# Atif-Anwer/SHMGAN

Hardware: AMD Instinct MI355X
Metric: images/sec (gen+disc train_step) (higher is better)
Workload: dtype f32; 1 GPU; SHMGAN train_step 256x256 5-view, batch 8/GPU, filter_size 64, fp32 (BASELINE configs[1]); global_batch=8, image_size=256, parallelism=dp1, losses_finite=True

## Files before the change

### shmgan_amd/csrc/conv_halo.hip

```cpp
#include "tapgemm_dev.h"

template <typename T, typename TO, int BN, int PH = 16, bool ST = false, int TM = 2, bool GS = false, int NM = 0>
__global__ __launch_bounds__(BN * PH / (2 * TM), ST ? BN * PH / (256 * TM) : 1) void tapgemm_halo_kernel(const TapGemmArgs a) {
    static_assert(TM == 2 || (TM == 4 && ST), "four M tiles per wave: static-tap form only");
    static_assert(!NM || (ST && TM == 2 && !GS), "norm: static-tap forward form");
    constexpr int ESZ = sizeof(T), CHE = 16 / ESZ, BKE = 64 / ESZ;
    constexpr int WGM = PH / (2 * TM), WGN = BN / 64, NW = WGM * WGN;
    constexpr int HC = 18, NIT = PH == 16 ? 24 : 12;
    constexpr int NHR = NIT * 16;
    constexpr int ASTG = NHR * 16, BSTG = BN * 16;
    constexpr int NA = NIT / NW, NB = (BN / 16) / NW;
    static_assert(NIT % NW == 0 && (BN / 16) % NW == 0, "DMA items divide over the waves");
    __shared__ __attribute__((aligned(1024))) float smem[2 * ASTG + 3 * BSTG];
    __shared__ __attribute__((aligned(1024))) float snt[NM ? SHM_NT_PLANES * SHM_NT_MAXC : 4];
    float* const sA = smem;
    float* const sB = smem + 2 * ASTG;
    typedef __attribute__((address_space(3))) void* lds_ptr;

    const TapPhase& P = a.ph[0];
    const int tid = threadIdx.x;
    const int lane = tid & 63, wave = __builtin_amdgcn_readfirstlane(tid >> 6);
    const int l31 = lane & 31, h = lane >> 5;
    const int wm = wave / WGN, wn = wave % WGN;
    const int ppr = a.wi >> 4, ppi = (a.hi / PH) * ppr;
    const int img = blockIdx.x / ppi, prem = blockIdx.x - img * ppi;
    const int y0 = (prem / ppr) * PH, x0 = (prem % ppr) << 4;
    const int n0 = blockIdx.y * BN;
    [[maybe_unused]] const bool nm_table = NM == 1 || (NM == 2 && (y0 == 0 || y0 + PH == a.hi || x0 == 0 || x0 + 16 == a.wi));

    const int drow = lane >> 2, dq = lane & 3;
    unsigned arow1[NA], arow2[NA];
    [[maybe_unused]] int nmv[NA];
#pragma unroll
    for (int j = 0; j < NA; ++j) {
        const int hrow = 16 * (wave + NW * j) + drow;
        const int hr = hrow / HC, hc = hrow - hr * HC;
        const int iy = y0 - 1 + hr, ix = x0 - 1 + hc;
        const bool v = hrow < (PH + 2) * HC && (unsigned)iy < (unsigned)a.hi && (unsigned)ix < (unsigned)a.wi;
        const int pix = (img * a.hi + iy) * a.wi + ix;
        const int coff = (dq ^ (ST ? ((hrow >> 1) + hr) & 3 : (hrow >> 2) & 3)) * CHE;
        arow1[j] = v ? (unsigned)(pix * a.ldx + coff) * (unsigned)ESZ : 0xffffffffu;
        arow2[j] = v ? (unsigned)(pix * a.ldx2 + coff) * (unsigned)ESZ : 0xffffffffu;
        nmv[j] = v ? coff : hrow < (PH + 2) * HC ? -1 - coff : (int)0x80000000;
    }
    unsigned wrow[NB];
#pragma unroll
    for (int j = 0; j < NB; ++j) {
        const int row = (wave + NW * j) * 16 + drow;
        const int nn = n0 + row;
        wrow[j] = nn < a.nout ? (unsigned)(nn * a.K + (dq ^ ((row >> 2) & 3)) * CHE) * (unsigned)ESZ : 0xffffffffu;
    }
    const __amdgpu_buffer_rsrc_t rsx = __builtin_amdgcn_make_buffer_rsrc((void*)a.x, 0, a.xbytes, 0x00020000);
    const __amdgpu_buffer_rsrc_t rsx2 = __builtin_amdgcn_make_buffer_rsrc((void*)a.x2, 0, a.x2bytes, 0x00020000);
    const __amdgpu_buffer_rsrc_t rsw = __builtin_amdgcn_make_buffer_rsrc((void*)a.w, 0, a.wbytes, 0x00020000);

    const int nch = a.K / BKE;
    const int ksteps = 9 * nch;
    const int tl = lane < 9 ? lane : 0;
    const int tapsh_v = P.dh[tl] * HC + P.dw[tl];
    const int tapw_v = P.widx[tl];

    auto dma_a = [&](int chunk) {
        const int c0 = chunk * BKE;
        const bool second = c0 >= a.c1;
        const unsigned cb = (unsigned)(second ? c0 - a.c1 : c0) * (unsigned)ESZ;
        float* dst = sA + (chunk & 1) * ASTG + wave * 256;
#pragma unroll
        for (int j = 0; j < NA; ++j) {
            const unsigned r = second ? arow2[j] : arow1[j];
            const unsigned off = r == 0xffffffffu ? r : r + cb;
            if (second)
                __builtin_amdgcn_raw_ptr_buffer_load_lds(rsx2, (lds_ptr)(dst + j * NW * 256), 16, (int)off, 0, 0, 0);
            else
                __builtin_amdgcn_raw_ptr_buffer_load_lds(rsx, (lds_ptr)(dst + j * NW * 256), 16, (int)off, 0, 0, 0);
        }
    };
    int ld_tap = 0, ld_chunk = 0, ld_stage = 0;
    auto dma_b = [&]() {
        const int t_wi = __builtin_amdgcn_readlane(tapw_v, ld_tap);
        const unsigned wbase = (unsigned)((t_wi * a.nout) * a.K + ld_chunk * BKE) * (unsigned)ESZ + (NM == 2 ? (unsigned)img * a.wimg : 0u);
#pragma unroll
        for (int j = 0; j < NB; ++j) {
            const unsigned off = wrow[j] == 0xffffffffu ? wrow[j] : wrow[j] + wbase;
            __builtin_amdgcn_raw_ptr_buffer_load_lds(rsw, (lds_ptr)(sB + ld_stage * BSTG + (wave + NW * j) * 256), 16, (int)off, 0, 0, 0);
        }
        if (++ld_tap == 9) {
            ld_tap = 0;
            ++ld_chunk;
        }
        ld_stage = ld_stage == 2 ? 0 : ld_stage + 1;
    };

    f32x16 acc[TM][2];
#pragma unroll
    for (int i = 0; i < TM; ++i)
#pragma unroll
        for (int j = 0; j < 2; ++j)
#pragma unroll
            for (int r = 0; r < 16; ++r) acc[i][j][r] = 0.f;

    int hb[TM];
#pragma unroll
    for (int i = 0; i < TM; ++i) hb[i] = (2 * TM * wm + 2 * i + (l31 >> 4) + 1) * HC + (l31 & 15) + 1;
    const int swb = (l31 >> 2) & 3;
    const int fb0 = l31 * 16 + ((0 + h) ^ swb) * 4, fb1 = l31 * 16 + ((2 + h) ^ swb) * 4;

    [[maybe_unused]] f32x4 abl_frag = {0.f, 0.f, 0.f, 0.f};
    if constexpr (abl::nolds) abl_frag = *(const f32x4*)(sA + lane * 4);
    auto compute = [&](int chunk, int tap, int bstage) {
        const float* Ab = sA + (chunk & 1) * ASTG;
        const float* Bb = sB + bstage * BSTG + wn * 64 * 16;
        const int sh = __builtin_amdgcn_readlane(tapsh_v, tap);
        int fa[2][2];
#pragma unroll
        for (int i = 0; i < 2; ++i) {
            const int hrow = hb[i] + sh;
            const int sw = (hrow >> 2) & 3;
            fa[i][0] = hrow * 16 + ((0 + h) ^ sw) * 4;
            fa[i][1] = hrow * 16 + ((2 + h) ^ sw) * 4;
        }
#pragma unroll
        for (int kk = 0; kk < 2; ++kk) {
            f32x4 av[2], bv[2];
            if constexpr (abl::nolds) {
                for (int i = 0; i < 2; ++i) av[i] = abl_frag;
                for (int j = 0; j < 2; ++j) bv[j] = abl_frag;
                asm volatile("" : "+v"(av[0]), "+v"(av[1]), "+v"(bv[0]), "+v"(bv[1]));
            } else {
#pragma unroll
                for (int i = 0; i < 2; ++i) av[i] = *(const f32x4*)(Ab + fa[i][kk]);
#pragma unroll
                for (int j = 0; j < 2; ++j) bv[j] = *(const f32x4*)(Bb + j * 512 + (kk ? fb1 : fb0));
            }
            if constexpr (TM == 2) tap_mfma<T, 2, 2>(av, bv, acc);
        }
    };

    [[maybe_unused]] int ntc_s = NM ? a.ntc : 0;
    if constexpr (NM != 0) asm volatile("" : "+s"(ntc_s));
    [[maybe_unused]] auto norm_a = [&](int chunk) {
        const int c0 = chunk * BKE;
        const bool second = c0 >= a.c1;
        if ((int)second != a.ntpart) return;
        const float* tb0 = snt + (second ? c0 - a.c1 : c0);
        float* dst = sA + (chunk & 1) * ASTG + wave * 256 + lane * 4;
        if constexpr (NM == 2) {
            if (!nm_table) return;
#pragma unroll
            for (int j = 0; j < NA; ++j) {
                const int m = nmv[j];
                if (m < 0 && m != (int)0x80000000) {
                    const float* tb = tb0 + (-1 - m) + 3 * ntc_s;
                    float* p = dst + j * NW * 256;
                    if constexpr (ESZ == 4) {
                        *(f32x4*)p = *(const f32x4*)tb;
                    } else {
                        const f32x4 r0 = *(const f32x4*)tb, r1 = *(const f32x4*)(tb + 4);
                        u32x4 x;
#pragma unroll
                        for (int e = 0; e < 2; ++e) {
                            x[e] = (unsigned)__builtin_bit_cast(unsigned short, (bf16_t)r0[2 * e]) |
                                   ((unsigned)__builtin_bit_cast(unsigned short, (bf16_t)r0[2 * e + 1]) << 16);
                            x[2 + e] = (unsigned)__builtin_bit_cast(unsigned short, (bf16_t)r1[2 * e]) |
                                       ((unsigned)__builtin_bit_cast(unsigned short, (bf16_t)r1[2 * e + 1]) << 16);
                        }
                        *(u32x4*)p = x;
                    }
                }
            }
            return;
        } else {
#pragma unroll
        for (int j = 0; j < NA; ++j) {
            if (nmv[j] >= 0) {
                const float* tb = tb0 + nmv[j];
                float* p = dst + j * NW * 256;
                if constexpr (ESZ == 4) {
                    f32x4 x = *(const f32x4*)p;
                    const f32x4 mean = *(const f32x4*)tb, inv = *(const f32x4*)(tb + ntc_s), beta = *(const f32x4*)(tb + 2 * ntc_s);
#pragma unroll
                    for (int e = 0; e < 4; ++e) x[e] = shm_in_norm(x[e], mean[e], inv[e], beta[e]);
                    *(f32x4*)p = x;
                } else {
                    u32x4 x = *(const u32x4*)p;
#pragma unroll
                    for (int hf = 0; hf < 2; ++hf) {
                        const f32x4 mean = *(const f32x4*)(tb + 4 * hf), inv = *(const f32x4*)(tb + ntc_s + 4 * hf),
                                    beta = *(const f32x4*)(tb + 2 * ntc_s + 4 * hf);
#pragma unroll
                        for (int e = 0; e < 2; ++e) {
                            const unsigned u = x[2 * hf + e];
                            const bf16_t lo = (bf16_t)shm_in_norm(__uint_as_float(u << 16), mean[2 * e], inv[2 * e], beta[2 * e]);
                            const bf16_t hi = (bf16_t)shm_in_norm(__uint_as_float(u & 0xffff0000u), mean[2 * e + 1], inv[2 * e + 1], beta[2 * e + 1]);
                            x[2 * hf + e] = (unsigned)__builtin_bit_cast(unsigned short, lo) | ((unsigned)__builtin_bit_cast(unsigned short, hi) << 16);
                        }
                    }
                    *(u32x4*)p = x;
                }
            }
        }
        }
    };

    if constexpr (NM) if (nm_table) {
        const __amdgpu_buffer_rsrc_t rsn = __builtin_amdgcn_make_buffer_rsrc((void*)a.nt, 0, a.ntbytes, 0x00020000);
        if (wave < SHM_NT_PLANES)
            __builtin_amdgcn_raw_ptr_buffer_load_lds(rsn, (lds_ptr)(snt + wave * 256), 16,
                                                     (int)((unsigned)img * 16u * (unsigned)a.ntc + (unsigned)wave * 1024u + (unsigned)lane * 16u), 0, 0, 0);
    }
    dma_a(0);
    dma_b();
    if (ksteps > 1) dma_b();
    if constexpr (NM) if (nm_table) {
        asm volatile("s_waitcnt vmcnt(%0)" ::"n"(2 * NB) : "memory");
        SHM_LDS_BARRIER();
        asm volatile("" ::: "memory");
        norm_a(0);
    }
    if constexpr (ST) {
        int fs[9];
#pragma unroll
        for (int t = 0; t < 9; ++t) {
            const int hrow = hb[0] + P.dh[t] * HC + P.dw[t];
            fs[t] = hrow * 16 + ((h ^ (((hrow >> 1) + hrow / HC) & 3)) << 2);
        }
        typedef const __attribute__((address_space(3))) f32x4* lds_f4;
        const unsigned sA_lds = (unsigned)(size_t)(__attribute__((address_space(3))) float*)sA;
        int tw[9];
#pragma unroll
        for (int t = 0; t < 9; ++t) tw[t] = __builtin_amdgcn_readlane(tapw_v, t);
        auto dma_b_at = [&](int t_wi, int chunk2, int stage2) {
            const unsigned wbase = (unsigned)((t_wi * a.nout) * a.K + chunk2 * BKE) * (unsigned)ESZ + (NM == 2 ? (unsigned)img * a.wimg : 0u);
#pragma unroll
            for (int j = 0; j < NB; ++j) {
                const unsigned off = wrow[j] == 0xffffffffu ? wrow[j] : wrow[j] + wbase;
                __builtin_amdgcn_raw_ptr_buffer_load_lds(rsw, (lds_ptr)(sB + stage2 * BSTG + (wave + NW * j) * 256), 16, (int)off, 0, 0, 0);
            }
        };
        for (int chunk = 0; chunk < nch; ++chunk) {
            const unsigned Ab = sA_lds + (unsigned)((chunk & 1) * ASTG * 4);
#pragma unroll
            for (int tap = 0; tap < 9; ++tap) {
                if (tap == 8 && chunk + 1 == nch)
                    asm volatile("s_waitcnt vmcnt(0)" ::: "memory");
                else if (tap == 1 && chunk + 1 < nch)
                    asm volatile("s_waitcnt vmcnt(%0)" ::"n"(NA + NB) : "memory");
                else
                    asm volatile("s_waitcnt vmcnt(%0)" ::"n"(NB) : "memory");
                SHM_LDS_BARRIER();
                asm volatile("" ::: "memory");
                if constexpr (!abl::nodma) {
                    if (tap == 0 && chunk + 1 < nch) dma_a(chunk + 1);
                    if (tap < 7 || chunk + 1 < nch) dma_b_at(tw[(tap + 2) % 9], chunk + (tap + 2) / 9, (tap + 2) % 3);
                }
                const float* Bb = sB + (tap % 3) * BSTG + wn * 64 * 16;
#pragma unroll
                for (int kk = 0; kk < 2; ++kk) {
                    f32x4 av[TM], bv[2];
                    if constexpr (abl::nolds) {
                        for (int i = 0; i < TM; ++i) av[i] = abl_frag;
                        for (int j = 0; j < 2; ++j) bv[j] = abl_frag;
                        asm volatile("" : "+v"(av[0]), "+v"(av[1]), "+v"(bv[0]), "+v"(bv[1]));
                    } else {
                        const lds_f4 ap = (lds_f4)(size_t)((Ab + (unsigned)(fs[tap] << 2)) ^ (unsigned)(kk << 5));
#pragma unroll
                        for (int i = 0; i < TM; ++i) av[i] = ap[i * (2 * HC * 4)];
#pragma unroll
                        for (int j = 0; j < 2; ++j) bv[j] = *(const f32x4*)(Bb + j * 512 + (kk ? fb1 : fb0));
                    }
                    if constexpr (!abl::nomfma)
                        tap_mfma<T, TM, 2>(av, bv, acc);
                    else
                        asm volatile("" :: "v"(av[0]), "v"(av[1]), "v"(bv[0]), "v"(bv[1]));
                }
                asm volatile("" ::: "memory");
                if constexpr (NM)
                    if (tap == 2 && chunk + 1 < nch && nm_table) {
                        norm_a(chunk + 1);
                        asm volatile("" ::: "memory");
                    }
            }
        }
    } else {
    int tap = 0, chunk = 0, bst = 0;
    for (int s = 0; s < ksteps; ++s) {
        if (s + 1 < ksteps) {
            if (tap == 1 && chunk + 1 < nch)
                asm volatile("s_waitcnt vmcnt(%0)" ::"n"(NA + NB) : "memory");
            else
                asm volatile("s_waitcnt vmcnt(%0)" ::"n"(NB) : "memory");
        } else {
            asm volatile("s_waitcnt vmcnt(0)" ::: "memory");
        }
        SHM_LDS_BARRIER();
        asm volatile("" ::: "memory");
        if constexpr (!abl::nodma) {
            if (tap == 0 && chunk + 1 < nch) dma_a(chunk + 1);
            if (s + 2 < ksteps) dma_b();
        }
        if constexpr (!abl::nomfma) compute(chunk, tap, bst);
        asm volatile("" ::: "memory");
        bst = bst == 2 ? 0 : bst + 1;
        if (++tap == 9) {
            tap = 0;
            ++chunk;
        }
    }
    }

    float s1[2], s2[2];
#pragma unroll
    for (int j = 0; j < 2; ++j) s1[j] = s2[j] = 0.f;
    float bj[2];
#pragma unroll
    for (int j = 0; j < 2; ++j) {
        const int n = n0 + wn * 64 + j * 32 + l31;
        bj[j] = (a.bias && n < a.nout) ? a.bias[(NM == 2 ? (size_t)img * a.bias_img : (size_t)0) + n] : 0.f;
        asm volatile("" : "+v"(bj[j]));
    }
    constexpr bool kWide = sizeof(TO) == 2;
    const bool wide = kWide && (a.nout % 8 == 0) && (a.n1 % 8 == 0) && (a.ldy % 8 == 0) && (((size_t)a.y & 15) == 0) &&
                      (a.y2 == nullptr || ((a.ldy2 % 8 == 0) && (((size_t)a.y2 & 15) == 0)));
    if constexpr (kWide) if (wide) {
        __syncthreads();
        unsigned short* tile = (unsigned short*)smem + wave * (TM * 32 * 64);
#pragma unroll
        for (int i = 0; i < TM; ++i) {
#pragma unroll
            for (int r = 0; r < 16; ++r) {
                const int row = i * 32 + (r & 3) + 8 * (r >> 2) + 4 * h;
#pragma unroll
                for (int j = 0; j < 2; ++j) {
                    const int n = n0 + wn * 64 + j * 32 + l31;
                    float v = acc[i][j][r] + bj[j];
                    const TO vo = (TO)shm_lrelu(v, a.slope);
                    v = n < a.nout ? (float)vo : 0.f;
                    s1[j] += v;
                    s2[j] = __builtin_fmaf(v, v, s2[j]);
                    const int col = j * 32 + l31;
                    tile[row * 64 + ((((col >> 3) ^ (row & 7)) << 3) | (col & 7))] = __builtin_bit_cast(unsigned short, vo);
                }
            }
        }
        asm volatile("s_waitcnt lgkmcnt(0)" ::: "memory");
        const int rr = lane >> 3, ch = lane & 7;
        const int n = n0 + wn * 64 + ch * 8;
        const int gp = __builtin_amdgcn_readfirstlane(n0 + wn * 64) < a.n1 ? 0 : 1;
        const int gpc = gp ? a.nout - a.n1 : a.n1, gnl = n - (gp ? a.n1 : 0);
        const bool gon = GS && a.gred[gp] != nullptr;
        const bool gs = gon && n < a.nout;
        const __amdgpu_buffer_rsrc_t rsa = __builtin_amdgcn_make_buffer_rsrc((void*)a.gaux[gp], 0, gon ? 0xfffffff0u : 0u, 0x00020000);
        const unsigned ldab = (unsigned)a.ldgaux[gp] * 2u;
        float t1[8], t2[8];
        u32x4 gav[4 * TM];
        if constexpr (GS) {
#pragma unroll
            for (int e = 0; e < 8; ++e) t1[e] = t2[e] = 0.f;
#pragma unroll
            for (int it = 0; it < 4 * TM; ++it) {
                const int row = it * 8 + rr;
                const int i = row >> 5, r32 = row & 31;
                const int py = 2 * TM * wm + 2 * i + (r32 >> 4), px = r32 & 15;
                const unsigned opix = (unsigned)((img * a.hi + (y0 + py)) * a.wi + (x0 + px));
                gav[it] = __builtin_bit_cast(u32x4, __builtin_amdgcn_raw_buffer_load_b128(rsa, opix * ldab + (unsigned)(n < a.nout ? gnl : 0) * 2u, 0, 0));
            }
            asm volatile("" ::: "memory");
        }
#pragma unroll
        for (int it = 0; it < 4 * TM; ++it) {
            const int row = it * 8 + rr;
            const u32x4 v = *(const u32x4*)(tile + row * 64 + ((ch ^ (row & 7)) << 3));
            const int i = row >> 5, r32 = row & 31;
            const int py = 2 * TM * wm + 2 * i + (r32 >> 4), px = r32 & 15;
            const size_t opix = ((size_t)img * a.hi + (y0 + py)) * a.wi + (x0 + px);
            if (!abl::nostore && n < a.nout) {
                if (n < a.n1)
                    *(u32x4*)((unsigned short*)a.y + opix * a.ldy + n) = v;
                else
                    *(u32x4*)((unsigned short*)a.y2 + opix * a.ldy2 + (n - a.n1)) = v;
            }
            if constexpr (GS) {
                gsum_wide_accum(v, gav[it], t1, t2);
                asm volatile("" ::: "memory");
            }
        }
        if constexpr (GS) {
            if (gon) {
                const int slot = (prem * WGM + wm) % a.gslots;
                double* dst = gs ? a.gred[gp] + ((size_t)slot * a.gbatch * gpc + (size_t)img * gpc + gnl) * 2 : nullptr;
                gsum_wide_flush<8>(t1, t2, lane, dst);
            }
        }
    }
    const bool gs_any = GS && sizeof(TO) == 4 && (a.gred[0] != nullptr || a.gred[1] != nullptr);
    if constexpr (GS && sizeof(TO) == 4) if (!wide && gs_any) {
#pragma unroll
        for (int j = 0; j < 2; ++j) {
            const int nb = __builtin_amdgcn_readfirstlane(n0 + wn * 64 + j * 32);
            const int gp = nb < a.n1 ? 0 : 1;
            const bool on = a.gred[gp] != nullptr && nb < a.nout;
            const int n = nb + l31;
            const int nl = n - (gp ? a.n1 : 0);
            const int pc = gp ? a.nout - a.n1 : a.n1;
            const __amdgpu_buffer_rsrc_t rsa = __builtin_amdgcn_make_buffer_rsrc((void*)a.gaux[gp], 0, on ? 0xfffffff0u : 0u, 0x00020000);
            const unsigned ldab = (unsigned)a.ldgaux[gp] * (unsigned)sizeof(T), nlb = (unsigned)(n < a.nout ? nl : 0) * (unsigned)sizeof(T);
            const __amdgpu_buffer_rsrc_t rsy = __builtin_amdgcn_make_buffer_rsrc(gp ? a.y2 : a.y, 0, gp ? a.y2bytes : a.ybytes, 0x00020000);
            const unsigned ldyb = (unsigned)(gp ? a.ldy2 : a.ldy) * (unsigned)sizeof(TO), nyb = (unsigned)(n < a.nout ? nl : 0) * (unsigned)sizeof(TO);
#pragma unroll
            for (int i = 0; i < TM; ++i) {
                const unsigned pix0 = (unsigned)((img * a.hi + (y0 + 2 * TM * wm + 2 * i)) * a.wi + x0 + 4 * h);
                const unsigned ao = pix0 * ldab + nlb, yo = pix0 * ldyb + nyb;
                float q[16];
#pragma unroll
                for (int r = 0; r < 16; ++r) {
                    const unsigned cr = (unsigned)((r >> 3) * a.wi + 8 * ((r >> 2) & 1) + (r & 3));
                    if constexpr (sizeof(T) == 4)
                        q[r] = __builtin_bit_cast(float, __builtin_amdgcn_raw_buffer_load_b32(rsa, ao, cr * ldab, 0));
                    else
                        q[r] = __uint_as_float((unsigned)__builtin_amdgcn_raw_buffer_load_b16(rsa, ao, cr * ldab, 0) << 16);
                }
                if (n < a.nout) {
#pragma unroll
                    for (int r = 0; r < 16; ++r) {
                        const unsigned cr = (unsigned)((r >> 3) * a.wi + 8 * ((r >> 2) & 1) + (r & 3));
                        float v = acc[i][j][r] + bj[j];
                        const TO vo = (TO)shm_lrelu(v, a.slope);
                        v = (float)vo;
                        s1[j] += v;
                        s2[j] += v * q[r];
                        __builtin_amdgcn_raw_buffer_store_b32(__builtin_bit_cast(unsigned, vo), rsy, yo, cr * ldyb, 0);
                    }
                }
            }
            if (on) {
                const int slot = (prem * WGM + wm) % a.gslots;
                const float t1 = s1[j] + __shfl_xor(s1[j], 32, 64);
                const float t2 = s2[j] + __shfl_xor(s2[j], 32, 64);
                if (h == 0 && n < a.nout) {
                    double* dst = a.gred[gp] + ((size_t)slot * a.gbatch * pc + (size_t)img * pc + nl) * 2;
                    atomicAdd(dst, (double)t1);
                    atomicAdd(dst + 1, (double)t2);
                }
            }
        }
    }
    const bool ybuf = !abl::nostore && a.ybytes != 0 && (a.y2 == nullptr || (a.y2bytes != 0 && a.n1 % 32 == 0));
    if (!wide && !gs_any && ybuf) {
#pragma unroll
        for (int j = 0; j < 2; ++j) {
            const int nb = __builtin_amdgcn_readfirstlane(n0 + wn * 64 + j * 32);
            const int gp = nb < a.n1 ? 0 : 1;
            const int n = nb + l31;
            const __amdgpu_buffer_rsrc_t rsy = __builtin_amdgcn_make_buffer_rsrc(gp ? a.y2 : a.y, 0, gp ? a.y2bytes : a.ybytes, 0x00020000);
            const unsigned ldyb = (unsigned)(gp ? a.ldy2 : a.ldy) * (unsigned)sizeof(TO);
            const unsigned nyb = (unsigned)(n < a.nout ? n - (gp ? a.n1 : 0) : 0) * (unsigned)sizeof(TO);
            if (n < a.nout) {
#pragma unroll
                for (int i = 0; i < TM; ++i) {
                    const unsigned yo = (unsigned)((img * a.hi + (y0 + 2 * TM * wm + 2 * i)) * a.wi + x0 + 4 * h) * ldyb + nyb;
#pragma unroll
                    for (int r = 0; r < 16; ++r) {
                        const unsigned cr = (unsigned)((r >> 3) * a.wi + 8 * ((r >> 2) & 1) + (r & 3));
                        float v = acc[i][j][r] + bj[j];
                        const TO vo = (TO)shm_lrelu(v, a.slope);
                        v = (float)vo;
                        s1[j] += v;
                        s2[j] = __builtin_fmaf(v, v, s2[j]);
                        if constexpr (sizeof(TO) == 4)
                            __builtin_amdgcn_raw_buffer_store_b32(__builtin_bit_cast(unsigned, vo), rsy, yo, cr * ldyb, 0);
                        else
                            __builtin_amdgcn_raw_buffer_store_b16(__builtin_bit_cast(unsigned short, vo), rsy, yo, cr * ldyb, 0);
                    }
                }
            }
        }
    }
    if (!wide && !gs_any && !ybuf) {
#pragma unroll
    for (int i = 0; i < TM; ++i) {
#pragma unroll
        for (int r = 0; r < 16; ++r) {
            const int row = (r & 3) + 8 * (r >> 2) + 4 * h;
            const int py = 2 * TM * wm + 2 * i + (row >> 4), px = row & 15;
            const size_t opix = ((size_t)img * a.hi + (y0 + py)) * a.wi + (x0 + px);
#pragma unroll
            for (int j = 0; j < 2; ++j) {
                const int n = n0 + wn * 64 + j * 32 + l31;
                if (n < a.nout) {
                    float v = acc[i][j][r] + bj[j];
                    const TO vo = (TO)shm_lrelu(v, a.slope);
                    v = (float)vo;
                    s1[j] += v;
                    s2[j] = __builtin_fmaf(v, v, s2[j]);
                    if (!abl::nostore || v == 123.456f)
                    {
                        if (n < a.n1)
                            ((TO*)a.y)[opix * a.ldy + n] = vo;
                        else
                            ((TO*)a.y2)[opix * a.ldy2 + (n - a.n1)] = vo;
                    }
                }
            }
        }
    }
    }
    if (a.stats) {
        const int slot = (prem * WGM + wm) % a.stats_slots;
#pragma unroll
        for (int j = 0; j < 2; ++j) {
            float t1 = s1[j] + __shfl_xor(s1[j], 32, 64);
            float t2 = s2[j] + __shfl_xor(s2[j], 32, 64);
            const int n = n0 + wn * 64 + j * 32 + l31;
            if (h == 0 && n < a.nout) {
                double* dst = a.stats + (size_t)slot * a.stats_stride + ((size_t)img * a.nout + n) * 2;
                atomicAdd(dst, (double)t1);
                atomicAdd(dst + 1, (double)t2);
            }
        }
    }
}

template <typename T, typename TO, int BN, int PH = 16, bool ST = false, int TM = 2, bool GS = false, int NM = 0>
static void halo_launch(const TapGemmArgs& a, int batch, hipStream_t st) {
    hipLaunchKernelGGL((tapgemm_halo_kernel<T, TO, BN, PH, ST, TM, GS, NM>), dim3(batch * (a.hi / PH) * (a.wi / 16), shm_cdiv(a.nout, BN), 1), dim3(BN * PH / (2 * TM)), 0, st, a);
    shm_set_last_kernel("tapgemm_halo_kernel<%s, %s, %d, %d, %s, %d%s>", shm_tg_name<T>(), shm_tg_name<TO>(), BN, PH, ST ? "true" : "false", TM,
                        NM == 2 ? ", false, 2" : NM == 1 ? ", false, 1" : GS ? ", true" : "");
}

template <typename T, typename TO, int BN>
static void halo_st_launch(const TapGemmArgs& a, const TapGemmPlan& p, int batch, hipStream_t st) {
    if (p.gs_fused)
        halo_launch<T, TO, BN, 16, true, 2, true>(a, batch, st);
    else if (a.nt) {
        if constexpr (sizeof(T) == sizeof(TO)) {
            if (a.ntmode)
                halo_launch<T, TO, BN, 16, true, 2, false, 2>(a, batch, st);
            else
                halo_launch<T, TO, BN, 16, true, 2, false, 1>(a, batch, st);
        }
    } else
        halo_launch<T, TO, BN, 16, true>(a, batch, st);
}

template <typename T, typename TO>
static int halo_launch_t(const TapGemmArgs& a, const TapGemmPlan& p, int batch, hipStream_t st, const char* who) {
    const int v = p.variant;
    SHM_REQUIRE(v != SHM_TG_HALO128_PH8 || (p.halo_ok && sizeof(T) == 2), SHM_E_SHAPE, "%s: forced variant halo128/ph8 is bf16, unit-stride 3x3, map multiple of 16", who);
    SHM_REQUIRE(p.halo_ok, SHM_E_SHAPE, "%s: forced variant %s needs a unit-stride 3x3 layer on a map that is a multiple of 16", who,
                v == SHM_TG_HALO128 ? "halo128" : v == SHM_TG_HALO64 ? "halo64" : v == SHM_TG_HALO128_ST ? "halo128/static-taps" : v == SHM_TG_HALO64_ST ? "halo64/static-taps"
                                                                                                                                   : "halo128/static-taps/4 waves");
// ... 19 lines not shown
```

### shmgan_amd/csrc/conv_igemm.hip

```cpp
#include "tapgemm.h"

struct ConvExtras {
    double* stats = nullptr;
    int stats_hw = 0, stats_slots = 1;
    const void* gaux[2] = {};
    int ldgaux[2] = {};
    double* gred[2] = {};
    ShmNormReq norm = {};
    bool gsum_fused = false;
};

static TapGemmPlan tapgemm_plan(const TapGemmArgs& a, int batch, int nphase, int esz, int oesz, bool two_src, bool want_norm) {
    const int BKE = 64 / esz;
    const int forced = shm_tune(SHM_TUNE_TAPGEMM_VARIANT);
    bool halo_ok = nphase == 1 && a.is == 1 && a.os == 1 && a.ph[0].ntaps == 9 && a.hi % 16 == 0 && a.wi % 16 == 0 && a.hg == a.hi && a.wg == a.wi;
    if (halo_ok)
        for (int t = 0; t < 9; ++t)
            halo_ok = halo_ok && a.ph[0].dh[t] >= -1 && a.ph[0].dh[t] <= 1 && a.ph[0].dw[t] >= -1 && a.ph[0].dw[t] <= 1;
    const bool bk32_ok = a.K % (2 * BKE) == 0 && (!two_src || a.c1 % (2 * BKE) == 0);
    const bool wreg_ok = esz == 2 && halo_ok && !two_src && (a.K == 32 || a.K == 64) && a.ybytes != 0 && (a.y2 == nullptr || a.y2bytes != 0) &&
                         a.slope >= 0.f && a.slope <= 1.f &&
                         (oesz == 4 || (a.nout % 64 == 0 && a.n1 % 32 == 0 && a.ldy % 8 == 0 && ((size_t)a.y & 15) == 0 &&
                                        (a.y2 == nullptr || (a.ldy2 % 8 == 0 && ((size_t)a.y2 & 15) == 0))));
    const int wreg32_wn = a.nout % 64 == 0 ? 4 : a.nout == 32 ? 2 : a.nout == 16 ? 1 : 0;
    const bool wreg32_ok = esz == 4 && oesz == 4 && halo_ok && (!two_src || (a.c1 == 16 && a.K == 32 && a.nout == 16)) && a.ybytes != 0 &&
                           (a.y2 == nullptr || a.y2bytes != 0) && a.slope >= 0.f && a.slope <= 1.f && a.n1 % 16 == 0 &&
                           ((wreg32_wn == 4 && (a.K == 16 || a.K == 32 || a.K == 64)) || (wreg32_wn == 2 && a.hi % 16 == 0 && (a.K == 16 || a.K == 32)) ||
                            (wreg32_wn == 1 && a.hi % 32 == 0 && (a.K == 16 || a.K == 32)));
    bool phase4_ok = nphase == 4 && a.is == 1 && a.os == 2 && !two_src && a.y2 == nullptr && a.stats == nullptr && a.hi % 16 == 0 &&
                     a.wi % 16 == 0 && a.hg == a.hi && a.wg == a.wi && a.ho == 2 * a.hi && a.wo == 2 * a.wi && a.nout % 64 == 0 &&
                     a.ph[0].ntaps == 4 && a.ph[1].ntaps == 2 && a.ph[2].ntaps == 2 && a.ph[3].ntaps == 1;
    if (phase4_ok)
        for (int p = 0; p < 4; ++p)
            for (int t = 0; t < a.ph[p].ntaps; ++t)
                phase4_ok = phase4_ok && a.ph[p].dh[t] >= -1 && a.ph[p].dh[t] <= 1 && a.ph[p].dw[t] >= -1 && a.ph[p].dw[t] <= 1;
    int v = forced;
    if (v == SHM_TG_AUTO) {
        const long tiles128 = (long)shm_cdiv(a.M, 128) * shm_cdiv(a.nout, 128) * nphase;
        if (wreg_ok || wreg32_ok) {
            v = SHM_TG_WREG;
        } else if (phase4_ok && (long)batch * (a.hi / 16) * (a.wi / 16) * (a.nout / 64) >= shm_tune(SHM_TUNE_TAPGEMM_PHASE4_MIN) &&
                   (esz == 2 || a.K <= 256)) {
            v = SHM_TG_PHASE4;
        } else if (halo_ok) {
            const long np16 = (long)batch * (a.hi / 16) * (a.wi / 16);
            const long nb128 = np16 * shm_cdiv(a.nout, 128), nb64 = np16 * shm_cdiv(a.nout, 64);
            auto fill = [](long nb) { return (double)nb / (double)(((nb + 511) / 512) * 512); };
            if (esz == 4 && nb64 < 256)
                v = SHM_TG_DMA_64x64;
            else if (a.nout <= 64)
                v = SHM_TG_HALO64_ST;
            else if (esz == 4 && nb128 < shm_tune(SHM_TUNE_TAPGEMM_HALO_MIN))
                v = (double)((nb128 + 255) / 256) <= (double)((nb64 + 255) / 256) * 0.52 ? SHM_TG_HALO128_ST : SHM_TG_HALO64_ST;
            else if (nb128 >= (esz == 2 ? 512 : shm_tune(SHM_TUNE_TAPGEMM_HALO_MIN)) || fill(nb128) * 1.03 >= fill(nb64))
                v = SHM_TG_HALO128_ST;
            else
                v = SHM_TG_HALO64_ST;
        } else if ((long)shm_cdiv(a.M, 64) * shm_cdiv(a.nout, 128) * nphase < 256) {
            v = SHM_TG_DMA_64x64;
        } else if (nphase == 1 && a.nout > 64 && a.K <= (esz == 2 ? 256 : 128) &&
                   (long)shm_cdiv(a.M, 256) * shm_cdiv(a.nout, 128) >= 256) {
            v = SHM_TG_DMA_256x128;
        } else if (nphase == 1 && a.nout > 64 && bk32_ok && (esz == 2 ? a.K >= 256 : (a.K >= 256 && a.K < 512 && a.is == 2 && tiles128 >= 512))) {
            v = SHM_TG_DMA_128x128_BK32;
        } else if (a.nout > 64 && tiles128 < shm_tune(SHM_TUNE_TAPGEMM_SMALL_GRID)) {
            v = SHM_TG_DMA_64x128;
        } else if (a.nout > 64) {
            v = SHM_TG_DMA_128x128;
        } else {
            v = SHM_TG_DMA_128x64;
        }
    }
    const bool want_gs = a.gred[0] || a.gred[1];
    bool gs_fused = false;
    if (want_gs) {
        bool al = true;
        for (int p = 0; p < 2; ++p)
            if (a.gred[p]) al = al && (oesz == 4 || (a.ldgaux[p] % 8 == 0 && ((size_t)a.gaux[p] & 15) == 0));
        al = al && (a.y2 == nullptr || a.n1 % 32 == 0);
        const bool small = a.ybytes != 0 && (a.y2 == nullptr || a.y2bytes != 0);
        const bool wide_ok = oesz == 4 || ((a.nout % 8 == 0) && (a.n1 % 8 == 0) && (a.ldy % 8 == 0) && (((size_t)a.y & 15) == 0) &&
                                           (a.y2 == nullptr || ((a.ldy2 % 8 == 0) && (((size_t)a.y2 & 15) == 0))));
        al = al && wide_ok;
        switch (v) {
        case SHM_TG_HALO128_ST: case SHM_TG_HALO64_ST:
            gs_fused = al && small && (a.y2 == nullptr || a.n1 % 64 == 0);
            break;
        case SHM_TG_DMA_128x128: case SHM_TG_DMA_64x128: case SHM_TG_DMA_128x64: case SHM_TG_DMA_64x64: case SHM_TG_DMA_256x64:
        case SHM_TG_DMA_256x128: case SHM_TG_DMA_128x128_BK32: case SHM_TG_DMA_128x128_NST4:
            gs_fused = al && (a.hg * a.wg) % 64 == 0;
            break;
        case SHM_TG_WREG:
            gs_fused = al && small && ((wreg_ok && oesz == 2) || (wreg32_ok && wreg32_wn == 4 && !two_src));
            break;
        case SHM_TG_PHASE4:
            gs_fused = oesz == 4 && small && a.gred[1] == nullptr;
            break;
        default:
            break;
        }
    }
    bool norm_ok = false;
    if (want_norm) {
        const int pc = a.ntpart ? a.K - a.c1 : a.c1;
        norm_ok = !want_gs && nphase == 1 && a.ntc == pc && pc % BKE == 0 && pc <= SHM_NT_MAXC && (a.ntpart == 0 || two_src);
        switch (v) {
        case SHM_TG_HALO128_ST: case SHM_TG_HALO64_ST:
            norm_ok = norm_ok && halo_ok && oesz == esz;
            break;
        case SHM_TG_WREG:
            norm_ok = norm_ok && a.ntpart == 0 && pc <= 64 && ((wreg_ok && oesz == 2) || (wreg32_ok && wreg32_wn == 4 && !two_src));
            break;
        default:
            norm_ok = false;
        }
    }
    const bool x3 = esz == 4 && oesz == 4 && shm_tune(SHM_TUNE_CONV_F32_SPLIT) == 1 && halo_ok && (!want_norm || a.ntmode == 0) &&
                    (v == SHM_TG_HALO128_ST || v == SHM_TG_HALO64_ST || (v == SHM_TG_WREG && forced == SHM_TG_AUTO)) && (!want_gs || gs_fused) && shm_x3_fwd_eligible(a);
    const int w16 = shm_tune(SHM_TUNE_TAPGEMM_WREG16);
    int wreg16 = 0;
    if (v == SHM_TG_WREG && wreg_ok && oesz == 2 && w16 != 0 && !gs_fused && !want_norm && a.nout % 64 == 0 && (a.y2 == nullptr || a.n1 % 64 == 0) && !two_src &&
        a.ybytes != 0 && (a.y2 == nullptr || a.y2bytes != 0))
        wreg16 = w16 == 2 && shm_pp_eligible(a) ? 2 : 1;
    return TapGemmPlan{v, gs_fused, norm_ok, halo_ok, bk32_ok, wreg_ok, wreg32_ok, phase4_ok, wreg32_wn, x3, wreg16};
}

static int finish_args(TapGemmArgs& a, int batch, int nphase, int dtype, bool two_src, const char* who, const ConvExtras& ex) {
    SHM_REQUIRE(dtype == SHM_F32 || dtype == SHM_BF16 || dtype == SHM_BF16_GF32, SHM_E_DTYPE,
                "%s: dtype %d not in {SHM_F32, SHM_BF16, SHM_BF16_GF32}", who, dtype);
    a.stats = ex.stats;
    a.hw = ex.stats_hw;
    a.stats_slots = ex.stats_slots;
    a.stats_stride = (unsigned)batch * (unsigned)a.nout * 2u;
    for (int p = 0; p < 2; ++p) {
        a.gaux[p] = ex.gaux[p];
        a.ldgaux[p] = ex.ldgaux[p];
        a.gred[p] = ex.gred[p];
    }
    a.gslots = SHM_GSUM_SLOTS;
    a.gbatch = batch;
    a.nt = ex.norm.nt;
    a.ntpart = ex.norm.part;
    a.ntc = ex.norm.c;
    a.ntmode = ex.norm.mode;
    a.ntbytes = (unsigned)((size_t)batch * SHM_NT_PLANES * ex.norm.c * sizeof(float));
    a.wimg = 0;
    a.bias_img = 0;
    if (a.gred[0] || a.gred[1]) {
        SHM_REQUIRE(a.stats == nullptr, SHM_E_SHAPE, "%s: fused forward statistics and gsum are exclusive", who);
        a.hw = a.hg * a.wg;
    }
    SHM_REQUIRE(dtype != SHM_BF16_GF32 || a.stats == nullptr, SHM_E_DTYPE, "%s: SHM_BF16_GF32 has no fused statistics", who);
    const int esz = dtype == SHM_F32 ? 4 : 2, bke = 64 / esz, che = 16 / esz;
    SHM_REQUIRE(a.K % bke == 0 && a.K > 0, SHM_E_SHAPE, "%s: contraction channels %d must be a multiple of %d", who, a.K, bke);
    SHM_REQUIRE(a.c1 % bke == 0, SHM_E_SHAPE, "%s: concat split %d must be a multiple of %d", who, a.c1, bke);
    SHM_REQUIRE(a.ldx % che == 0 && (!two_src || a.ldx2 % che == 0), SHM_E_SHAPE, "%s: input pitch must be a multiple of 16 bytes", who);
    SHM_REQUIRE(((size_t)a.x & 15) == 0 && ((size_t)a.x2 & 15) == 0, SHM_E_SHAPE, "%s: input tensors must be 16-byte aligned", who);
    const bool compact_rgb = !two_src && a.ldx * esz == 16 && a.K * esz == 64;
    SHM_REQUIRE(compact_rgb || a.ldx >= a.c1, SHM_E_SHAPE, "%s: input pitch %d below the source's %d channels", who, a.ldx, a.c1);
    SHM_REQUIRE(!two_src || a.ldx2 >= a.K - a.c1, SHM_E_SHAPE, "%s: input pitch %d of the second source below its %d channels", who, a.ldx2, a.K - a.c1);
    SHM_REQUIRE(a.ldy >= a.n1, SHM_E_SHAPE, "%s: output pitch %d below the part's %d channels", who, a.ldy, a.n1);
    SHM_REQUIRE(a.y2 == nullptr || a.ldy2 >= a.nout - a.n1, SHM_E_SHAPE, "%s: output pitch %d of the second part below its %d channels", who, a.ldy2, a.nout - a.n1);
    for (int p = 0; p < 2; ++p)
        SHM_REQUIRE(a.gred[p] == nullptr || a.ldgaux[p] >= (p ? a.nout - a.n1 : a.n1), SHM_E_SHAPE, "%s: aux pitch %d below the part's %d channels", who,
                    a.ldgaux[p], p ? a.nout - a.n1 : a.n1);
    SHM_REQUIRE((size_t)batch * a.hi * a.wi < (1u << 31) && (size_t)batch * a.ho * a.wo < (1u << 31), SHM_E_SHAPE, "%s: pixel count overflows int32", who);
    a.M = batch * a.hg * a.wg;
    if (a.M == 0 || a.nout == 0) return SHM_OK;
    {
        const size_t lim = 0xfffffff0ull;
        size_t xb = (size_t)batch * a.hi * a.wi * a.ldx * esz, x2b = two_src ? (size_t)batch * a.hi * a.wi * a.ldx2 * esz : 0;
        size_t wb = 0;
        for (int p = 0; p < nphase; ++p)
            for (int t = 0; t < a.ph[p].ntaps; ++t) {
                size_t e = (size_t)(a.ph[p].widx[t] + 1) * a.nout * a.K * esz;
                if (e > wb) wb = e;
            }
        if (a.nt && a.ntmode) {
            SHM_REQUIRE(nphase == 1 && a.bias, SHM_E_SHAPE, "%s: SHM_NORM_SCALED takes per-sample weights AND per-sample bias rows", who);
            a.wimg = (unsigned)((size_t)a.ph[0].ntaps * a.nout * a.K * esz);
            a.bias_img = a.nout;
            wb = (size_t)batch * a.wimg;
        }
        SHM_REQUIRE(xb < lim && x2b < lim && wb < lim, SHM_E_SHAPE, "%s: operand larger than 4 GiB (32-bit buffer offsets)", who);
        a.xbytes = (unsigned)xb;
        a.x2bytes = (unsigned)x2b;
        a.wbytes = (unsigned)wb;
        const int oesz = dtype == SHM_BF16 ? 2 : 4;
        const size_t yb = (size_t)batch * a.ho * a.wo * a.ldy * oesz, y2b = a.y2 ? (size_t)batch * a.ho * a.wo * a.ldy2 * oesz : 0;
        const bool flat = shm_tune(SHM_TUNE_TAPGEMM_FLAT_EPILOGUE) != 0;
        a.ybytes = (yb < lim && !flat) ? (unsigned)yb : 0u;
        a.y2bytes = (y2b < lim && !flat) ? (unsigned)y2b : 0u;
    }
    return SHM_OK;
}

static int device_cus() {
    static const int ncu = [] {
        int dev = 0, n = 0;
        if (hipGetDevice(&dev) != hipSuccess || hipDeviceGetAttribute(&n, hipDeviceAttributeMultiprocessorCount, dev) != hipSuccess || n <= 0) n = 256;
        return n;
    }();
    return ncu;
}

static int launch_plan(const TapGemmArgs& a, const TapGemmPlan& p, int batch, int nphase, int dtype, hipStream_t st, const char* who) {
    if (p.x3) return shm_x3_fwd_launch(a, batch, p.gs_fused, st, who);
    switch (p.variant) {
    case SHM_TG_HALO128: case SHM_TG_HALO64: case SHM_TG_HALO128_ST: case SHM_TG_HALO128_ST_W4: case SHM_TG_HALO64_ST: case SHM_TG_HALO128_PH8:
        return shm_halo_launch(a, p, batch, dtype, st, who);
    case SHM_TG_PHASE4:
        return shm_phase4_launch(a, p, batch, dtype, st, who);
    case SHM_TG_WREG: {
        SHM_REQUIRE(p.wreg_ok || p.wreg32_ok, SHM_E_SHAPE,
                    "%s: forced variant wreg needs a unit-stride 3x3 layer on a map that is a multiple of 16, slope in [0,1] and: bf16 -- one source "
                    "tensor with 32/64 channels, Cout %% 64 == 0; fp32 -- one source with 16/32/64 input channels and "
                    "Cout %% 64 == 0, or 16/32 input channels with Cout = 32 (map a multiple of 16) or 16 (map a multiple of 32; also 16 + 16 from two tensors)", who);
        const int np8 = batch * (a.hi / 8) * (a.wi / 16), ncu = device_cus();
        if (p.wreg16 == 2) return shm_pp_launch(a, batch, ncu, st, who);
        if (p.wreg16 == 1) return shm_wreg16_launch(a, np8, ncu, st, who);
        return p.wreg_ok ? shm_wreg_launch(a, p, np8, ncu, dtype, st, who) : shm_wreg_f32_launch(a, p, batch, ncu, st, who);
    }
    case SHM_TG_DMA_128x128: case SHM_TG_DMA_64x128: case SHM_TG_DMA_128x64: case SHM_TG_DMA_64x64: case SHM_TG_DMA_256x64:
    case SHM_TG_DMA_256x128: case SHM_TG_DMA_128x128_BK32: case SHM_TG_DMA_128x128_NST4:
        return shm_dma_launch(a, p, nphase, dtype, st, who);
    default:
        SHM_REQUIRE(false, SHM_E_SHAPE, "%s: unknown tapgemm.variant %d", who, p.variant);
    }
    return SHM_OK;
}

static int launch_tapgemm(TapGemmArgs& a, int batch, int nphase, int dtype, hipStream_t st, const char* who, ConvExtras& ex) {
    const bool two_src = a.x2 != nullptr;
    if (const int r = finish_args(a, batch, nphase, dtype, two_src, who, ex)) return r;
    if (a.M == 0 || a.nout == 0) return SHM_OK;
    const int esz = dtype == SHM_F32 ? 4 : 2, oesz = dtype == SHM_BF16 ? 2 : 4;
    if (nphase == 1 && a.is == 2 && a.os == 1 && a.ph[0].ntaps == 9 && a.ph[0].dh[0] == 0 && a.ph[0].dw[0] == 0 && !a.x2 && !a.y2 && !a.gred[0] && !a.gred[1] &&
        !a.nt && a.ldx * esz == 16 && a.K * esz == 64 && a.ybytes != 0 && dtype != SHM_BF16_GF32 &&
        shm_tune(SHM_TUNE_TAPGEMM_VARIANT) == SHM_TG_AUTO) {
        const int r = shm_rgb_s2_fwd_launch(a.x, a.ldx, a.w, a.K, a.bias, a.y, a.ldy, batch, a.hi, a.wi, a.nout, a.slope, a.stats, a.stats_slots, a.stats_stride,
                                            a.xbytes, a.ybytes, dtype, st);
        if (r < 0) return r;
        if (r == 1) return SHM_OK;
    }
    const TapGemmPlan p = tapgemm_plan(a, batch, nphase, esz, oesz, two_src, a.nt != nullptr);
    ex.gsum_fused = p.gs_fused;
    if (!p.gs_fused) a.gred[0] = a.gred[1] = nullptr;
    SHM_REQUIRE(a.nt == nullptr || p.norm_ok, SHM_E_SHAPE,
                "%s: the kernel this shape runs on (tapgemm variant %d) cannot normalise its source in LDS (unit-stride 3x3 on a map that is a "
                "multiple of 16, normalised part of at most %d channels; ask shm_conv2d_norm_supported) -- use shm_in_apply", who, p.variant, SHM_NT_MAXC);
    if (const int r = launch_plan(a, p, batch, nphase, dtype, st, who)) return r;
    SHM_LAUNCH_CHECK(who);
    return SHM_OK;
}

template <typename T>
__global__ void transpose_taps_kernel(const float* __restrict__ w, T* __restrict__ wt, int rows, int cols, int rows_pad) {
    __shared__ float tile[32][33];
    const int t = blockIdx.z;
    const int r0 = blockIdx.y * 32, c0 = blockIdx.x * 32;
    const float* src = w + (size_t)t * rows * cols;
    T* dst = wt + (size_t)t * cols * rows_pad;
    for (int i = threadIdx.y; i < 32; i += blockDim.y) {
        int r = r0 + i, c = c0 + threadIdx.x;
        tile[i][threadIdx.x] = (r < rows && c < cols) ? src[(size_t)r * cols + c] : 0.f;
    }
    __syncthreads();
    for (int i = threadIdx.y; i < 32; i += blockDim.y) {
        int c = c0 + i, r = r0 + threadIdx.x;
        if (c < cols && r < rows_pad) dst[(size_t)c * rows_pad + r] = (T)tile[threadIdx.x][i];
    }
}

extern "C" int shm_transpose_taps(const float* w, void* wt, int ntaps, int rows, int cols, int rows_pad, int dtype, void* stream) {
    SHM_REQUIRE(rows_pad >= rows && ntaps > 0 && rows > 0 && cols > 0, SHM_E_SHAPE, "shm_transpose_taps: bad shape");
    SHM_REQUIRE(dtype == SHM_F32 || dtype == SHM_BF16, SHM_E_DTYPE, "shm_transpose_taps: bad dtype %d", dtype);
    dim3 grid(shm_cdiv(cols, 32), shm_cdiv(rows_pad, 32), ntaps);
    if (dtype == SHM_BF16)
        hipLaunchKernelGGL(transpose_taps_kernel<bf16_t>, grid, dim3(32, 8), 0, (hipStream_t)stream, w, (bf16_t*)wt, rows, cols, rows_pad);
    else
        hipLaunchKernelGGL(transpose_taps_kernel<float>, grid, dim3(32, 8), 0, (hipStream_t)stream, w, (float*)wt, rows, cols, rows_pad);
    SHM_LAUNCH_CHECK("shm_transpose_taps");
    return SHM_OK;
}

constexpr int kMaxTransposes = 48;
struct TransposeBatch {
    const float* w[kMaxTransposes];
    void* wt[kMaxTransposes];
    int rows[kMaxTransposes], cols[kMaxTransposes], rows_pad[kMaxTransposes];
    int tx[kMaxTransposes], ty[kMaxTransposes];
    int block0[kMaxTransposes + 1];
    int count;
};

template <typename T>
__global__ void transpose_taps_multi_kernel(const TransposeBatch b) {
    __shared__ float tile[32][33];
    int l = 0;
    while (l + 1 < b.count && (int)blockIdx.x >= b.block0[l + 1]) ++l;
    const int rows = b.rows[l], cols = b.cols[l], rows_pad = b.rows_pad[l];
    int rem = (int)blockIdx.x - b.block0[l];
    const int per_tap = b.tx[l] * b.ty[l];
    const int t = rem / per_tap;
    rem -= t * per_tap;
    const int r0 = (rem / b.tx[l]) * 32, c0 = (rem % b.tx[l]) * 32;
    const float* src = b.w[l] + (size_t)t * rows * cols;
    T* dst = (T*)b.wt[l] + (size_t)t * cols * rows_pad;
    for (int i = threadIdx.y; i < 32; i += blockDim.y) {
        int r = r0 + i, c = c0 + threadIdx.x;
        tile[i][threadIdx.x] = (r < rows && c < cols) ? src[(size_t)r * cols + c] : 0.f;
    }
    __syncthreads();
    for (int i = threadIdx.y; i < 32; i += blockDim.y) {
        int c = c0 + i, r = r0 + threadIdx.x;
        if (c < cols && r < rows_pad) dst[(size_t)c * rows_pad + r] = (T)tile[threadIdx.x][i];
    }
}

extern "C" int shm_transpose_taps_multi(int count, const void* const* w, void* const* wt, const int* ntaps, const int* rows, const int* cols,
                                        const int* rows_pad, int dtype, void* stream) {
    SHM_REQUIRE(count >= 0 && count <= kMaxTransposes, SHM_E_SHAPE, "shm_transpose_taps_multi: %d layers (at most %d)", count, kMaxTransposes);
    SHM_REQUIRE(dtype == SHM_F32 || dtype == SHM_BF16, SHM_E_DTYPE, "shm_transpose_taps_multi: bad dtype %d", dtype);
    if (count == 0) return SHM_OK;
    SHM_REQUIRE(w && wt && ntaps && rows && cols && rows_pad, SHM_E_SHAPE, "shm_transpose_taps_multi: null table");
    TransposeBatch b{};
    b.count = count;
    int total = 0;
    for (int l = 0; l < count; ++l) {
        SHM_REQUIRE(w[l] && wt[l] && rows_pad[l] >= rows[l] && ntaps[l] > 0 && rows[l] > 0 && cols[l] > 0, SHM_E_SHAPE,
                    "shm_transpose_taps_multi: bad shape of layer %d", l);
        b.w[l] = (const float*)w[l];
        b.wt[l] = wt[l];
        b.rows[l] = rows[l];
        b.cols[l] = cols[l];
        b.rows_pad[l] = rows_pad[l];
        b.tx[l] = shm_cdiv(cols[l], 32);
        b.ty[l] = shm_cdiv(rows_pad[l], 32);
        b.block0[l] = total;
        total += ntaps[l] * b.tx[l] * b.ty[l];
    }
    b.block0[count] = total;
    if (dtype == SHM_BF16)
        hipLaunchKernelGGL(transpose_taps_multi_kernel<bf16_t>, dim3(total), dim3(32, 8), 0, (hipStream_t)stream, b);
    else
        hipLaunchKernelGGL(transpose_taps_multi_kernel<float>, dim3(total), dim3(32, 8), 0, (hipStream_t)stream, b);
    SHM_LAUNCH_CHECK("shm_transpose_taps_multi");
    return SHM_OK;
}

template <typename T>
__global__ __launch_bounds__(256) void norm_prepare_kernel(const T* __restrict__ wk, const float* __restrict__ bias, const float* __restrict__ nt, int c,
                                                           int part_lo, T* __restrict__ wk_n, float* __restrict__ bias_n, int ntaps, int cout, int K) {
    const int co = blockIdx.x, n = blockIdx.y;
    const float* mean = nt + (size_t)n * SHM_NT_PLANES * c;
    const float *inv = mean + c, *beta = mean + 2 * c;
    float acc = 0.f;
// ... 279 lines not shown
```

Baseline: 70.04 images/sec.

## Shrink halo64 static-tap LDS footprint to fit three waves per SIMD

For the BN=64, PH=16 static-tap halo kernel, the A staging buffer is sized to the exact halo (18x18 rows) rather than a rounded-up item count. The last wave loads one extra partial item row to cover the remainder. The norm table moves into the same shared allocation, and launch bounds request three waves per SIMD, aiming for higher occupancy and better latency hiding. The heuristic's fill model is updated so the 64-wide variant counts 768 resident slots. This costs a per-wave vmcnt special case and more register pressure under the tighter launch bound.

Measured after the change: 70.17 images/sec (median of 6 runs). No clear change (+0.2%).

```diff
diff --git a/shmgan_amd/csrc/conv_halo.hip b/shmgan_amd/csrc/conv_halo.hip
--- a/shmgan_amd/csrc/conv_halo.hip
+++ b/shmgan_amd/csrc/conv_halo.hip
@@ -1,18 +1,27 @@
 #include "tapgemm_dev.h"
 
+
+constexpr int halo_waves_per_simd(int BN, int PH, bool ST, int TM, bool GS, int NM, int osz) {
+    return !ST ? 1 : BN == 64 && PH == 16 && TM == 2 && NM == 0 && !(GS && osz == 2) ? 3 : BN * PH / (256 * TM);
+}
+
 template <typename T, typename TO, int BN, int PH = 16, bool ST = false, int TM = 2, bool GS = false, int NM = 0>
-__global__ __launch_bounds__(BN * PH / (2 * TM), ST ? BN * PH / (256 * TM) : 1) void tapgemm_halo_kernel(const TapGemmArgs a) {
+__global__ __launch_bounds__(BN * PH / (2 * TM), halo_waves_per_simd(BN, PH, ST, TM, GS, NM, sizeof(TO))) void tapgemm_halo_kernel(const TapGemmArgs a) {
     static_assert(TM == 2 || (TM == 4 && ST), "four M tiles per wave: static-tap form only");
     static_assert(!NM || (ST && TM == 2 && !GS), "norm: static-tap forward form");
     constexpr int ESZ = sizeof(T), CHE = 16 / ESZ, BKE = 64 / ESZ;
     constexpr int WGM = PH / (2 * TM), WGN = BN / 64, NW = WGM * WGN;
+    constexpr bool XA = ST && BN == 64 && PH == 16 && TM == 2;
     constexpr int HC = 18, NIT = PH == 16 ? 24 : 12;
-    constexpr int NHR = NIT * 16;
+    constexpr int NHR = XA ? (PH + 2) * HC : NIT * 16;
     constexpr int ASTG = NHR * 16, BSTG = BN * 16;
-    constexpr int NA = NIT / NW, NB = (BN / 16) / NW;
-    static_assert(NIT % NW == 0 && (BN / 16) % NW == 0, "DMA items divide over the waves");
-    __shared__ __attribute__((aligned(1024))) float smem[2 * ASTG + 3 * BSTG];
-    __shared__ __attribute__((aligned(1024))) float snt[NM ? SHM_NT_PLANES * SHM_NT_MAXC : 4];
+    constexpr int XROW = NHR - 16;
+    constexpr int NA = XA ? NHR / (16 * NW) + 1 : NIT / NW, NB = (BN / 16) / NW;
+    static_assert(XA ? NHR / 16 % NW == 0 && NHR % 16 != 0 : NIT % NW == 0, "DMA items divide over the waves");
+    static_assert((BN / 16) % NW == 0, "DMA items divide over the waves");
+    constexpr int SNT = 2 * ASTG + 3 * BSTG;
+    __shared__ __attribute__((aligned(1024))) float smem[SNT + (NM ? SHM_NT_PLANES * SHM_NT_MAXC : 0)];
+    [[maybe_unused]] float* const snt = smem + SNT;
     float* const sA = smem;
     float* const sB = smem + 2 * ASTG;
     typedef __attribute__((address_space(3))) void* lds_ptr;
@@ -31,9 +40,11 @@
     const int drow = lane >> 2, dq = lane & 3;
     unsigned arow1[NA], arow2[NA];
     [[maybe_unused]] int nmv[NA];
+    auto a_slot = [&](int j) { return XA && j == NA - 1 ? XROW * 16 : (wave + NW * j) * 256; };
 #pragma unroll
     for (int j = 0; j < NA; ++j) {
-        const int hrow = 16 * (wave + NW * j) + drow;
+        const bool extra = XA && j == NA - 1;
+        const int hrow = extra ? XROW + drow : 16 * (wave + NW * j) + drow;
         const int hr = hrow / HC, hc = hrow - hr * HC;
         const int iy = y0 - 1 + hr, ix = x0 - 1 + hc;
         const bool v = hrow < (PH + 2) * HC && (unsigned)iy < (unsigned)a.hi && (unsigned)ix < (unsigned)a.wi;
@@ -41,7 +52,8 @@
         const int coff = (dq ^ (ST ? ((hrow >> 1) + hr) & 3 : (hrow >> 2) & 3)) * CHE;
         arow1[j] = v ? (unsigned)(pix * a.ldx + coff) * (unsigned)ESZ : 0xffffffffu;
         arow2[j] = v ? (unsigned)(pix * a.ldx2 + coff) * (unsigned)ESZ : 0xffffffffu;
-        nmv[j] = v ? coff : hrow < (PH + 2) * HC ? -1 - coff : (int)0x80000000;
+        const bool mine = !extra || (wave == NW - 1 && hrow >= XROW + 16 - NHR % 16);
+        nmv[j] = !mine ? (int)0x80000000 : v ? coff : hrow < (PH + 2) * HC ? -1 - coff : (int)0x80000000;
     }
     unsigned wrow[NB];
 #pragma unroll
@@ -64,15 +76,16 @@
         const int c0 = chunk * BKE;
         const bool second = c0 >= a.c1;
         const unsigned cb = (unsigned)(second ? c0 - a.c1 : c0) * (unsigned)ESZ;
-        float* dst = sA + (chunk & 1) * ASTG + wave * 256;
+        float* dst = sA + (chunk & 1) * ASTG;
 #pragma unroll
         for (int j = 0; j < NA; ++j) {
+            if (XA && j == NA - 1 && wave != NW - 1) break;
             const unsigned r = second ? arow2[j] : arow1[j];
             const unsigned off = r == 0xffffffffu ? r : r + cb;
             if (second)
-                __builtin_amdgcn_raw_ptr_buffer_load_lds(rsx2, (lds_ptr)(dst + j * NW * 256), 16, (int)off, 0, 0, 0);
+                __builtin_amdgcn_raw_ptr_buffer_load_lds(rsx2, (lds_ptr)(dst + a_slot(j)), 16, (int)off, 0, 0, 0);
             else
-                __builtin_amdgcn_raw_ptr_buffer_load_lds(rsx, (lds_ptr)(dst + j * NW * 256), 16, (int)off, 0, 0, 0);
+                __builtin_amdgcn_raw_ptr_buffer_load_lds(rsx, (lds_ptr)(dst + a_slot(j)), 16, (int)off, 0, 0, 0);
         }
     };
     int ld_tap = 0, ld_chunk = 0, ld_stage = 0;
@@ -143,7 +156,7 @@
         const bool second = c0 >= a.c1;
         if ((int)second != a.ntpart) return;
         const float* tb0 = snt + (second ? c0 - a.c1 : c0);
-        float* dst = sA + (chunk & 1) * ASTG + wave * 256 + lane * 4;
+        float* dst = sA + (chunk & 1) * ASTG + lane * 4;
         if constexpr (NM == 2) {
             if (!nm_table) return;
 #pragma unroll
@@ -151,7 +164,7 @@
                 const int m = nmv[j];
                 if (m < 0 && m != (int)0x80000000) {
                     const float* tb = tb0 + (-1 - m) + 3 * ntc_s;
-                    float* p = dst + j * NW * 256;
+                    float* p = dst + a_slot(j);
                     if constexpr (ESZ == 4) {
                         *(f32x4*)p = *(const f32x4*)tb;
                     } else {
@@ -174,7 +187,7 @@
         for (int j = 0; j < NA; ++j) {
             if (nmv[j] >= 0) {
                 const float* tb = tb0 + nmv[j];
-                float* p = dst + j * NW * 256;
+                float* p = dst + a_slot(j);
                 if constexpr (ESZ == 4) {
                     f32x4 x = *(const f32x4*)p;
                     const f32x4 mean = *(const f32x4*)tb, inv = *(const f32x4*)(tb + ntc_s), beta = *(const f32x4*)(tb + 2 * ntc_s);
@@ -243,9 +256,12 @@
             for (int tap = 0; tap < 9; ++tap) {
                 if (tap == 8 && chunk + 1 == nch)
                     asm volatile("s_waitcnt vmcnt(0)" ::: "memory");
-                else if (tap == 1 && chunk + 1 < nch)
-                    asm volatile("s_waitcnt vmcnt(%0)" ::"n"(NA + NB) : "memory");
-                else
+                else if (tap == 1 && chunk + 1 < nch) {
+                    if (!XA || wave == NW - 1)
+                        asm volatile("s_waitcnt vmcnt(%0)" ::"n"(NA + NB) : "memory");
+                    else
+                        asm volatile("s_waitcnt vmcnt(%0)" ::"n"(NA - 1 + NB) : "memory");
+                } else
                     asm volatile("s_waitcnt vmcnt(%0)" ::"n"(NB) : "memory");
                 SHM_LDS_BARRIER();
                 asm volatile("" ::: "memory");
diff --git a/shmgan_amd/csrc/conv_igemm.hip b/shmgan_amd/csrc/conv_igemm.hip
--- a/shmgan_amd/csrc/conv_igemm.hip
+++ b/shmgan_amd/csrc/conv_igemm.hip
@@ -45,14 +45,14 @@
         } else if (halo_ok) {
             const long np16 = (long)batch * (a.hi / 16) * (a.wi / 16);
             const long nb128 = np16 * shm_cdiv(a.nout, 128), nb64 = np16 * shm_cdiv(a.nout, 64);
-            auto fill = [](long nb) { return (double)nb / (double)(((nb + 511) / 512) * 512); };
+            auto fill = [](long nb, long slots) { return (double)nb / (double)(((nb + slots - 1) / slots) * slots); };
             if (esz == 4 && nb64 < 256)
                 v = SHM_TG_DMA_64x64;
             else if (a.nout <= 64)
                 v = SHM_TG_HALO64_ST;
             else if (esz == 4 && nb128 < shm_tune(SHM_TUNE_TAPGEMM_HALO_MIN))
                 v = (double)((nb128 + 255) / 256) <= (double)((nb64 + 255) / 256) * 0.52 ? SHM_TG_HALO128_ST : SHM_TG_HALO64_ST;
-            else if (nb128 >= (esz == 2 ? 512 : shm_tune(SHM_TUNE_TAPGEMM_HALO_MIN)) || fill(nb128) * 1.03 >= fill(nb64))
+            else if (nb128 >= (esz == 2 ? 512 : shm_tune(SHM_TUNE_TAPGEMM_HALO_MIN)) || fill(nb128, 512) * 1.03 >= fill(nb64, 768))
                 v = SHM_TG_HALO128_ST;
             else
                 v = SHM_TG_HALO64_ST;
```
